# pmcbride/denoise-gan

Hardware: AMD Instinct MI355X
Metric: training images/sec, pix2pix 256x256 bs16/GPU (higher is better)
Workload: dtype fp32 (GEMMs fp16x3, operands 2^-22); 1 GPU; pix2pix train_step (train_pix2pix.py:33-71): G(x)+G(y) identity pass, D real+fake, GAN/L1/L2/TV/identity losses, D and G gradients, Keras Adam G and D; VGG19 content loss (seeded stand-in weights: ImageNet weights are a download); model=pix2pix U-Net G (54.4M) + PatchGAN D (2.77M), global_batch=16, batch_per_gpu=16, image_size=256, scale=1, parallelism=dp1, hip_graph=True, identity_pass=True

## Files before the change

denoise-gan_amd/csrc/conv.hip:

```cpp
#include "conv_plan.h"
#include "conv_tiles.h"
#include <algorithm>
#include <cstdlib>
#include <cstring>
#include <new>

namespace dg {

template <int MODE, int BM, int BN, int WGM, int WGN, bool VEC, int BK, int MINW>
__global__ void __launch_bounds__(256, MINW)
k_conv_gemm(const GemmArgs p) {
    constexpr bool A_KC = (MODE != MODE_WGRAD);
    constexpr bool B_KC = (MODE == MODE_DGRAD);
    constexpr int LDA = A_KC ? BM + 1 : BM + 4;
    constexpr int LDB = B_KC ? BN + 1 : BN + 4;
    constexpr int ASZ = BK * LDA;
    constexpr int BSZ = BK * LDB;
    constexpr int WTM = BM / WGM, WTN = BN / WGN;
    constexpr int TM = WTM / 32, TN = WTN / 32;
    static_assert(WGM * WGN == 4, "4 waves");
    static_assert(TM >= 1 && TN >= 1, "wave tile >= 32x32");
    static_assert(BK % 4 == 0 && BM >= 256 / (BK / 4) && BN >= 256 / (BK / 4), "KC loader geometry");
    static_assert(1024 / BM <= BK && 1024 / BN <= BK, "RC loader geometry");

// ... 242 lines not shown
                    *reinterpret_cast<f32x4 *>(&As[(ar_kr + AR_RPP * ip) * LDA + 4 * ar_c4]) = v;
                }
            } else {
#pragma unroll
                for (int e = 0; e < AR_NES; ++e) As[(as_kr + (256 / BM) * e) * LDA + as_c] = ra[e];
            }
        }
        if constexpr (B_KC) {
            if constexpr (VEC) {
#pragma unroll
                for (int ip = 0; ip < B_NPV; ++ip)
#pragma unroll
                    for (int q = 0; q < 4; ++q) Bs[(4 * kc_c4 + q) * LDB + kc_rr + KC_RPP * ip] = rb[4 * ip + q];
            } else {
#pragma unroll
                for (int e = 0; e < B_NES; ++e) Bs[ks_kk * LDB + ks_r0 + KS_RPP * e] = rb[e];
            }
        } else {
#pragma unroll
            for (int ip = 0; ip < BR_NP; ++ip) {
                f32x4 v = {rb[4 * ip], rb[4 * ip + 1], rb[4 * ip + 2], rb[4 * ip + 3]};
                *reinterpret_cast<f32x4 *>(&Bs[(br_kr + BR_RPP * ip) * LDB + 4 * br_c4]) = v;
            }
        }
    };

    f32x16 acc[TM][TN];
#pragma unroll
    for (int a = 0; a < TM; ++a)
#pragma unroll
        for (int b = 0; b < TN; ++b)
#pragma unroll
            for (int r = 0; r < 16; ++r) acc[a][b][r] = 0.f;

    load_tiles(kbeg);
    store_tiles(0);
    if (nk > 1) load_tiles(kbeg + BK);
    __syncthreads();

    for (int kt = 0; kt < nk; ++kt) {
        const int buf = kt & 1;
        const float *As = smem + buf * (ASZ + BSZ) + h2 * LDA + wm * WTM + l32;
        const float *Bs = smem + buf * (ASZ + BSZ) + ASZ + h2 * LDB + wn * WTN + l32;
        float af[BK / 2][TM], bf[BK / 2][TN];
#pragma unroll
        for (int s2 = 0; s2 < BK / 2; ++s2) {
#pragma unroll
            for (int a = 0; a < TM; ++a) af[s2][a] = As[2 * s2 * LDA + a * 32];
#pragma unroll
            for (int b = 0; b < TN; ++b) bf[s2][b] = Bs[2 * s2 * LDB + b * 32];
        }
        __builtin_amdgcn_sched_barrier(0);
#pragma unroll
        for (int s2 = 0; s2 < BK / 4; ++s2)
#pragma unroll
            for (int a = 0; a < TM; ++a)
#pragma unroll
                for (int b = 0; b < TN; ++b)
                    acc[a][b] = __builtin_amdgcn_mfma_f32_32x32x2f32(af[s2][a], bf[s2][b], acc[a][b], 0, 0, 0);
        __builtin_amdgcn_sched_barrier(0);
        if (kt + 1 < nk) store_tiles(buf ^ 1);
        if (kt + 2 < nk) load_tiles(kbeg + (kt + 2) * BK);
        __builtin_amdgcn_sched_barrier(0);
#pragma unroll
        for (int s2 = BK / 4; s2 < BK / 2; ++s2)
#pragma unroll
            for (int a = 0; a < TM; ++a)
#pragma unroll
                for (int b = 0; b < TN; ++b)
                    acc[a][b] = __builtin_amdgcn_mfma_f32_32x32x2f32(af[s2][a], bf[s2][b], acc[a][b], 0, 0, 0);
        __syncthreads();
    }

    static_assert(4 * 32 * 36 <= 2 * (ASZ + BSZ), "epilogue staging fits in the operand tiles");
    auto rowmap = [&](int row) __attribute__((always_inline)) -> RowPix {
        if (row >= Mrows) return RowPix{-1, -1};
        if constexpr (MODE == MODE_DGRAD) {
            int ww = row % ph.Wp; int t = row / ph.Wp; int hh = t % ph.Hp; int n = t / ph.Hp;
            return RowPix{row, (long)(n * g.H + hh * g.sh + ph.ph) * g.W + ww * g.sw + ph.pw};
        } else {
            return RowPix{row, row};
        }
    };
    conv_epilogue32<MODE, TM, TN>(p, acc, m0 + wm * WTM, n0 + wn * WTN, rowmap, phase, split, lane, smem + wid * 32 * 36);
}

template <int MODE>
__global__ void __launch_bounds__(256)
k_splitk_reduce(const GemmArgs p, int V4) {
    const ConvGeom &g = p.g;
    const int phase = blockIdx.y;
    int Mrows = p.M;
    PhaseInfo ph{};
    if constexpr (MODE == MODE_DGRAD) {
        ph = phase_info(g, phase, g.N);
        Mrows = ph.Mp;
    }
    const long plane = (long)p.M * p.N;
    const float *base = p.slab + (long)phase * p.splits * plane;
    const float ys = p.yp ? plane_scale(p) : 0.f;
    float vmax = 0.f;
    if (V4) {
        const int tpo = V4, opb = 256 / tpo;
        const int o = threadIdx.x % opb, j = threadIdx.x / opb;
        __shared__ f32x4 red[256];
        const int N4 = p.N >> 2;
        const long total = (long)Mrows * N4;
        const long step = (long)tpo * plane;
        for (long e0 = (long)blockIdx.x * opb; e0 < total; e0 += (long)gridDim.x * opb) {
            const long e = e0 + o;
            f32x4 v = {0.f, 0.f, 0.f, 0.f};
            int row = 0, col = 0;
            if (e < total) {
                row = (int)(e / N4);
                col = (int)(e - (long)row * N4) * 4;
                const float *src = base + (long)row * p.N + col + (long)j * plane;
                int s = j;
                for (; s + 3 * tpo < p.splits; s += 4 * tpo, src += 4 * step) {
                    const f32x4 a0 = *reinterpret_cast<const f32x4 *>(src);
                    const f32x4 a1 = *reinterpret_cast<const f32x4 *>(src + step);
                    const f32x4 a2 = *reinterpret_cast<const f32x4 *>(src + 2 * step);
                    const f32x4 a3 = *reinterpret_cast<const f32x4 *>(src + 3 * step);
                    v += a0;
                    v += a1;
                    v += a2;
                    v += a3;
                }
                for (; s < p.splits; s += tpo, src += step) v += *reinterpret_cast<const f32x4 *>(src);
            }
            if (tpo > 1) {
                red[threadIdx.x] = v;
                __syncthreads();
                if (j == 0)
                    for (int k = 1; k < tpo; ++k) v += red[k * opb + o];
                __syncthreads();
            }
            if (j != 0 || e >= total) continue;
            long pix;
            if constexpr (MODE == MODE_DGRAD) {
                int ww = row % ph.Wp; int t = row / ph.Wp; int hh = t % ph.Hp; int n = t / ph.Hp;
                pix = (long)(n * g.H + hh * g.sh + ph.ph) * g.W + ww * g.sw + ph.pw;
            } else {
                pix = row;
            }
            const long off = pix * p.ldc;
            f32x4 ov, mf;
#pragma unroll
            for (int q = 0; q < 4; ++q) {
                float x = v[q];
                if (p.bias) x += p.bias[col + q];
                mf[q] = epi_mask_factor(p, pix, col + q);
                ov[q] = act_fwd(x, p.act, p.alpha) * mf[q];
            }
            if (p.C) {
                f32x4 *dst = reinterpret_cast<f32x4 *>(p.C + off + col);
                if (p.beta != 0.f) ov += p.beta * (p.mask_acc ? (*dst) * mf : (*dst));
                *dst = ov;
            }
            if (p.yp) store_planes4(p.yp, p.ypC, pix, col, ov, ys);
#pragma unroll
            for (int q = 0; q < 4; ++q) vmax = fmaxf(vmax, fabsf(ov[q]));
        }
        if (p.ymax) block_atomic_absmax(p.ymax, vmax);
        return;
    }
    const long total = (long)Mrows * p.N;
    for (long e = (long)blockIdx.x * blockDim.x + threadIdx.x; e < total; e += (long)gridDim.x * blockDim.x) {
        int row = (int)(e / p.N);
        int col = (int)(e - (long)row * p.N);
        float v = 0.f;
        for (int s = 0; s < p.splits; ++s) v += base[s * plane + (long)row * p.N + col];
        long pix;
        if constexpr (MODE == MODE_DGRAD) {
            int ww = row % ph.Wp; int t = row / ph.Wp; int hh = t % ph.Hp; int n = t / ph.Hp;
            pix = (long)(n * g.H + hh * g.sh + ph.ph) * g.W + ww * g.sw + ph.pw;
        } else {
            pix = row;
        }
        const long off = pix * p.ldc;
        if (p.bias) v += p.bias[col];
        const float mf = epi_mask_factor(p, pix, col);
        v = act_fwd(v, p.act, p.alpha) * mf;
        if (p.C) {
            if (p.beta != 0.f) v += p.beta * (p.mask_acc ? p.C[off + col] * mf : p.C[off + col]);
            p.C[off + col] = v;
        }
        if (p.yp) store_planes1(p.yp, p.ypC, pix, col, v, ys);
        vmax = fmaxf(vmax, fabsf(v));
    }
    if (p.ymax) block_atomic_absmax(p.ymax, vmax);
}

constexpr int NARROW_MAX = 8;

__global__ void __launch_bounds__(256)
k_narrow_fwd(const GemmArgs p) {
    const ConvGeom &g = p.g;
    const int lane = threadIdx.x & 63;
    const int m = blockIdx.x * 4 + (threadIdx.x >> 6);
    if (m >= p.M) return;
    int wo = m % g.Wo; int t = m / g.Wo; int ho = t % g.Ho; int n = t / g.Ho;
    float acc[NARROW_MAX] = {};
    const int Co = g.Co;
    for (int i = 0; i < g.kh; ++i) {
        int hi = ho * g.sh - g.pt + i;
        if (hi < 0 || hi >= g.H) continue;
        for (int j = 0; j < g.kw; ++j) {
            int wi = wo * g.sw - g.pl + j;
            if (wi < 0 || wi >= g.W) continue;
            const float *xp = p.A + ((long)(n * g.H + hi) * g.W + wi) * p.lda;
            const float *wp = p.B + (long)(i * g.kw + j) * g.Ci * Co;
            for (int ci = lane; ci < g.Ci; ci += 64) {
                float xv = xp[ci];
#pragma unroll
                for (int co = 0; co < NARROW_MAX; ++co)
                    if (co < Co) acc[co] += xv * wp[(long)ci * Co + co];
            }
        }
    }
#pragma unroll
    for (int co = 0; co < NARROW_MAX; ++co) {
        float v = acc[co];
#pragma unroll
        for (int off = 32; off >= 1; off >>= 1) v += __shfl_xor(v, off);
        acc[co] = v;
    }
    if (lane == 0) {
        for (int co = 0; co < Co; ++co) {
            float v = acc[co];
            if (p.bias) v += p.bias[co];
            v = epi_mask(p, m, co, act_fwd(v, p.act, p.alpha));
            long off = (long)m * p.ldc + co;
            if (p.beta != 0.f) v += p.beta * p.C[off];
            p.C[off] = v;
        }
    }
}

__global__ void __launch_bounds__(256)
k_narrow_dgrad(const GemmArgs p, int w_in_lds) {
    extern __shared__ __attribute__((aligned(16))) float wl[];
    const ConvGeom &g = p.g;
    const int phase = blockIdx.y;
    PhaseInfo ph = phase_info(g, phase, g.N);
    const long wsz = (long)g.kh * g.kw * g.Ci * g.Co;
    const float *wsrc = p.B;
    if (w_in_lds) {
        for (long e = threadIdx.x; e < wsz; e += blockDim.x) wl[e] = p.B[e];
        __syncthreads();
        wsrc = wl;
    }
    const int m = blockIdx.x * blockDim.x + threadIdx.x;
    if (m >= ph.Mp) return;
    int ww = m % ph.Wp; int t = m / ph.Wp; int hh = t % ph.Hp; int n = t / ph.Hp;
    const int h = hh * g.sh + ph.ph, w = ww * g.sw + ph.pw;
    const int Ci = g.Ci, Co = g.Co;
    float acc[NARROW_MAX] = {};
    for (int a = 0; a < g.Th; ++a) {
        int i = ph.i0h + a * g.sh;
        int th = h + g.pt - i;
        if (i >= g.kh || th < 0) continue;
        int ho = th / g.sh;
        if (ho >= g.Ho) continue;
        for (int b = 0; b < g.Tw; ++b) {
            int j = ph.i0w + b * g.sw;
            int tw = w + g.pl - j;
            if (j >= g.kw || tw < 0) continue;
            int wo = tw / g.sw;
            if (wo >= g.Wo) continue;
            const float *dyp = p.A + ((long)(n * g.Ho + ho) * g.Wo + wo) * p.lda;
            const float *wp = wsrc + (long)(i * g.kw + j) * Ci * Co;
            if ((Co & 3) == 0 && (p.lda & 3) == 0) {
                for (int co = 0; co < Co; co += 4) {
                    f32x4 d = *reinterpret_cast<const f32x4 *>(dyp + co);
#pragma unroll
                    for (int ci = 0; ci < NARROW_MAX; ++ci) {
                        if (ci < Ci) {
                            const float *wr = wp + (long)ci * Co + co;
                            acc[ci] += d[0] * wr[0] + d[1] * wr[1] + d[2] * wr[2] + d[3] * wr[3];
                        }
                    }
                }
            } else {
                for (int co = 0; co < Co; ++co) {
                    float d = dyp[co];
#pragma unroll
                    for (int ci = 0; ci < NARROW_MAX; ++ci)
                        if (ci < Ci) acc[ci] += d * wp[(long)ci * Co + co];
                }
            }
        }
    }
    const long pix = (long)(n * g.H + h) * g.W + w;
    long off = pix * p.ldc;
    for (int ci = 0; ci < Ci; ++ci) {
        float v = acc[ci];
        if (p.bias) v += p.bias[ci];
        v = epi_mask(p, pix, ci, act_fwd(v, p.act, p.alpha));
        if (p.beta != 0.f) v += p.beta * p.C[off + ci];
        p.C[off + ci] = v;
    }
}


template <int CI, int TH, int TW>
__global__ void __launch_bounds__(256)
k_direct_dgrad(const GemmArgs p, int tiles_x, int tiles_y) {
    constexpr int HH = DIR_PH + TH - 1, HW = DIR_PW + TW - 1;
    __shared__ __attribute__((aligned(16))) float hal[HH * HW * DIR_CS];
    __shared__ __attribute__((aligned(16))) float wl[TH * TW * CI * DIR_CC];
    const ConvGeom &g = p.g;
    const int nph = g.sh * g.sw;
    const PhaseInfo ph = phase_info(g, blockIdx.x % nph, g.N);
    int t = blockIdx.x / nph;
    const int tx = t % tiles_x;
    t /= tiles_x;
    const int ty = t % tiles_y;
    const int n = t / tiles_y;
    const int hh0 = ty * DIR_PH, ww0 = tx * DIR_PW;
    if (hh0 >= ph.Hp || ww0 >= ph.Wp) return;
    const int oh = (ph.ph + g.pt - ph.i0h) / g.sh, ow = (ph.pw + g.pl - ph.i0w) / g.sw;
    const int ho0 = hh0 + oh - (TH - 1), wo0 = ww0 + ow - (TW - 1);
    const int lr = threadIdx.x / DIR_PW, lc = threadIdx.x % DIR_PW;
    float acc[CI];
#pragma unroll
    for (int ci = 0; ci < CI; ++ci) acc[ci] = 0.f;
    constexpr int NE = HH * HW * (DIR_CC / 4), NL = (NE + 255) / 256;
    f32x4 hv[NL];
    auto load_halo = [&](int c0) __attribute__((always_inline)) {
#pragma unroll
        for (int k = 0; k < NL; ++k) {
            const int e = threadIdx.x + 256 * k;
            hv[k] = f32x4{0.f, 0.f, 0.f, 0.f};
            if (e < NE) {
                const int q = e % (DIR_CC / 4), px = e / (DIR_CC / 4);
                const int r = px / HW, c = px - r * HW;
                const int ho = ho0 + r, wo = wo0 + c;
                if ((unsigned)ho < (unsigned)g.Ho && (unsigned)wo < (unsigned)g.Wo)
                    hv[k] = *reinterpret_cast<const f32x4 *>(p.A + ((long)(n * g.Ho + ho) * g.Wo + wo) * p.lda + c0 +
                                                             4 * q);
            }
        }
    };
    load_halo(0);
    for (int c0 = 0; c0 < g.Co; c0 += DIR_CC) {
        __syncthreads();
#pragma unroll
        for (int k = 0; k < NL; ++k) {
            const int e = threadIdx.x + 256 * k;
            if (e < NE) {
                const int q = e % (DIR_CC / 4), px = e / (DIR_CC / 4);
                *reinterpret_cast<f32x4 *>(&hal[px * DIR_CS + 4 * q]) = hv[k];
            }
        }
        for (int e = threadIdx.x; e < TH * TW * CI * DIR_CC; e += 256) {
            const int cc = e % DIR_CC, k = e / DIR_CC;
            const int ci = k % CI, tap = k / CI;
            const int i = ph.i0h + (tap / TW) * g.sh, j = ph.i0w + (tap % TW) * g.sw;
            wl[e] = (i < g.kh && j < g.kw) ? p.B[((long)(i * g.kw + j) * g.Ci + ci) * g.Co + c0 + cc] : 0.f;
        }
        __syncthreads();
        if (c0 + DIR_CC < g.Co) load_halo(c0 + DIR_CC);
#pragma unroll
        for (int a = 0; a < TH; ++a)
#pragma unroll
            for (int b = 0; b < TW; ++b) {
                const float *hp = &hal[((lr + TH - 1 - a) * HW + (lc + TW - 1 - b)) * DIR_CS];
                const float *wp = &wl[(a * TW + b) * CI * DIR_CC];
#pragma unroll
                for (int q = 0; q < DIR_CC / 4; ++q) {
                    const f32x4 d = *reinterpret_cast<const f32x4 *>(hp + 4 * q);
#pragma unroll
                    for (int ci = 0; ci < CI; ++ci) {
                        const f32x4 w = *reinterpret_cast<const f32x4 *>(wp + ci * DIR_CC + 4 * q);
                        float v = acc[ci];
                        v = fmaf(d[0], w[0], v);
                        v = fmaf(d[1], w[1], v);
                        v = fmaf(d[2], w[2], v);
                        v = fmaf(d[3], w[3], v);
                        acc[ci] = v;
                    }
                }
            }
    }
    const int hh = hh0 + lr, ww = ww0 + lc;
    if (hh >= ph.Hp || ww >= ph.Wp) return;
    const long pix = (long)(n * g.H + hh * g.sh + ph.ph) * g.W + ww * g.sw + ph.pw;
    const long off = pix * p.ldc;
#pragma unroll
    for (int ci = 0; ci < CI; ++ci) {
        float v = acc[ci];
        if (p.bias) v += p.bias[ci];
        v = epi_mask(p, pix, ci, act_fwd(v, p.act, p.alpha));
        if (p.beta != 0.f) v += p.beta * p.C[off + ci];
        p.C[off + ci] = v;
    }
}

static void launch_direct_dgrad(const GemmArgs &a, hipStream_t s) {
    const ConvGeom &g = a.g;
    const int Hp = (g.H + g.sh - 1) / g.sh, Wp = (g.W + g.sw - 1) / g.sw;
    const int tx = (Wp + DIR_PW - 1) / DIR_PW, ty = (Hp + DIR_PH - 1) / DIR_PH;
    const dim3 grid((unsigned)(g.N * tx * ty * g.sh * g.sw));
    if (g.Ci == 3 && g.Th == 3) hipLaunchKernelGGL((k_direct_dgrad<3, 3, 3>), grid, dim3(256), 0, s, a, tx, ty);
    else if (g.Ci == 3) hipLaunchKernelGGL((k_direct_dgrad<3, 2, 2>), grid, dim3(256), 0, s, a, tx, ty);
    else hipLaunchKernelGGL((k_direct_dgrad<6, 2, 2>), grid, dim3(256), 0, s, a, tx, ty);
}

constexpr int NFWD_WMAX = 8192;
constexpr long NFWD_PX_MIN_M = 4096;
template <int CO>
__global__ void __launch_bounds__(256)
k_narrow_fwd_px(const GemmArgs p) {
    __shared__ __attribute__((aligned(16))) float wl[NFWD_WMAX];
    const ConvGeom &g = p.g;
    const int ci4 = g.Ci / 4, ntap = g.kh * g.kw;
    for (int e = threadIdx.x; e < ntap * g.Ci * CO; e += 256) {
        const int q = e & 3, co = (e >> 2) % CO, rest = (e >> 2) / CO;
        const int c4 = rest % ci4, tap = rest / ci4;
        wl[e] = p.B[((long)tap * g.Ci + c4 * 4 + q) * CO + co];
    }
    __syncthreads();
    for (int m = blockIdx.x * 256 + threadIdx.x; m < p.M; m += gridDim.x * 256) {
        const int wo = m % g.Wo, t = m / g.Wo, ho = t % g.Ho, n = t / g.Ho;
        float acc[CO];
#pragma unroll
        for (int co = 0; co < CO; ++co) acc[co] = 0.f;
        for (int i = 0; i < g.kh; ++i) {
            const int hi = ho * g.sh - g.pt + i;
            if (hi < 0 || hi >= g.H) continue;
            for (int j = 0; j < g.kw; ++j) {
                const int wi = wo * g.sw - g.pl + j;
                if (wi < 0 || wi >= g.W) continue;
                const f32x4 *xp = reinterpret_cast<const f32x4 *>(p.A + ((long)(n * g.H + hi) * g.W + wi) * p.lda);
                const f32x4 *wp = reinterpret_cast<const f32x4 *>(wl) + (long)(i * g.kw + j) * ci4 * CO;
#pragma unroll 4
                for (int c = 0; c < ci4; ++c) {
                    const f32x4 x = xp[c];
#pragma unroll
                    for (int co = 0; co < CO; ++co) {
                        const f32x4 w = wp[c * CO + co];
                        acc[co] = fmaf(x[0], w[0], fmaf(x[1], w[1], fmaf(x[2], w[2], fmaf(x[3], w[3], acc[co]))));
                    }
                }
            }
        }
#pragma unroll
        for (int co = 0; co < CO; ++co) {
            float v = acc[co];
            if (p.bias) v += p.bias[co];
            v = epi_mask(p, m, co, act_fwd(v, p.act, p.alpha));
            const long off = (long)m * p.ldc + co;
            if (p.beta != 0.f) v += p.beta * p.C[off];
            p.C[off] = v;
        }
    }
}

__global__ void __launch_bounds__(256)
k_narrow_wgrad(const GemmArgs p) {
    __shared__ float red[256 * NARROW_MAX];
    const ConvGeom &g = p.g;
    const int nchunk = (g.Ci + 255) / 256;
    const int tap = blockIdx.x / nchunk;
    const int cchunk = blockIdx.x - tap * nchunk;
    int CL = 1;
    while (CL < g.Ci - cchunk * 256 && CL < 256) CL <<= 1;
    const int PL = 256 / CL;
    const int cl = threadIdx.x % CL, pl = threadIdx.x / CL;
    const int ci = cchunk * 256 + cl;
    const bool cok = ci < g.Ci;
    const int split = blockIdx.y;
    const int i = tap / g.kw, j = tap - (tap / g.kw) * g.kw;
    const int Co = g.Co;
    const int pb = split * p.kchunk, pe = min(p.K, pb + p.kchunk);
    float acc[NARROW_MAX] = {};
    constexpr int U = 4;
    int wo = (pb + pl) % g.Wo, ho = ((pb + pl) / g.Wo) % g.Ho, n = (pb + pl) / (g.Wo * g.Ho);
    auto advance = [&]() __attribute__((always_inline)) {
        wo += PL;
        if (wo >= g.Wo) {
            const int q = wo / g.Wo;
            wo -= q * g.Wo;
            ho += q;
            if (ho >= g.Ho) {
                const int q2 = ho / g.Ho;
                ho -= q2 * g.Ho;
                n += q2;
            }
        }
    };
    for (int pix0 = pb + pl; pix0 < pe; pix0 += U * PL) {
        float xv[U], dv[U][NARROW_MAX];
#pragma unroll
        for (int u = 0; u < U; ++u) {
            const int pix = pix0 + u * PL;
            xv[u] = 0.f;
#pragma unroll
            for (int co = 0; co < NARROW_MAX; ++co) dv[u][co] = 0.f;
            const int hi = ho * g.sh - g.pt + i, wi = wo * g.sw - g.pl + j, nn = n;
            advance();
            if (pix >= pe) continue;
            if (!cok || hi < 0 || hi >= g.H || wi < 0 || wi >= g.W) continue;
            xv[u] = p.A[((long)(nn * g.H + hi) * g.W + wi) * p.lda + ci];
            const float *dyp = p.B + (long)pix * p.ldb;
#pragma unroll
            for (int co = 0; co < NARROW_MAX; ++co)
                if (co < Co) dv[u][co] = dyp[co];
        }
#pragma unroll
        for (int u = 0; u < U; ++u)
#pragma unroll
            for (int co = 0; co < NARROW_MAX; ++co) acc[co] += xv[u] * dv[u][co];
    }
#pragma unroll
    for (int co = 0; co < NARROW_MAX; ++co) red[threadIdx.x * NARROW_MAX + co] = acc[co];
    __syncthreads();
    if (pl != 0 || !cok) return;
    for (int l = 1; l < PL; ++l)
#pragma unroll
        for (int co = 0; co < NARROW_MAX; ++co) acc[co] += red[(threadIdx.x + l * CL) * NARROW_MAX + co];
    const int krow = tap * g.Ci + ci;
    for (int co = 0; co < Co; ++co)
        p.slab[((long)split * p.M + krow) * p.N + co] = acc[co];
}


__global__ void __launch_bounds__(256)
k_narrow_wgrad_tile(const GemmArgs p, int nseg, float *__restrict__ part) {
    extern __shared__ __attribute__((aligned(16))) float sm[];
    const ConvGeom &g = p.g;
    const int Ci = g.Ci, KW = g.kw, KH = g.kh, Co = g.Co;
    const int CG = (Co + 3) >> 2;
    const int XW = NWT_TP + KW - 1;
    const int XE = KH * XW * Ci;
    float *xs = sm;
    f32x4 *ds = reinterpret_cast<f32x4 *>(sm + ((XE + 3) & ~3));
    const bool xv4 = (Ci & 3) == 0 && (p.lda & 3) == 0 && (((uintptr_t)p.A) & 15) == 0;
    const bool dv4 = (Co & 3) == 0 && (p.ldb & 3) == 0 && (((uintptr_t)p.B) & 15) == 0;
    const int S = KH * KW * Ci * CG;
    const int segw = (g.Wo + NWT_TP - 1) / NWT_TP;
    f32x4 acc[NWT_QMAX];
#pragma unroll
    for (int u = 0; u < NWT_QMAX; ++u) acc[u] = f32x4{0.f, 0.f, 0.f, 0.f};
    for (int seg = blockIdx.x; seg < nseg; seg += gridDim.x) {
        const int sx = seg % segw, t = seg / segw;
        const int ho = t % g.Ho, n = t / g.Ho;
        const int wo0 = sx * NWT_TP;
        if (xv4) {
            const int ci4 = Ci >> 2;
            for (int e = threadIdx.x; e < XE / 4; e += 256) {
                const int c4 = e % ci4, r = e / ci4;
                const int col = r % XW, i = r / XW;
                const int hi = ho - g.pt + i, wi = wo0 - g.pl + col;
                f32x4 v = {0.f, 0.f, 0.f, 0.f};
                if ((unsigned)hi < (unsigned)g.H && (unsigned)wi < (unsigned)g.W)
                    v = *reinterpret_cast<const f32x4 *>(p.A + ((long)(n * g.H + hi) * g.W + wi) * p.lda + 4 * c4);
                reinterpret_cast<f32x4 *>(xs)[e] = v;
            }
        } else {
            for (int e = threadIdx.x; e < XE; e += 256) {
                const int c = e % Ci, r = e / Ci;
                const int col = r % XW, i = r / XW;
                const int hi = ho - g.pt + i, wi = wo0 - g.pl + col;
                xs[e] = ((unsigned)hi < (unsigned)g.H && (unsigned)wi < (unsigned)g.W)
                            ? p.A[((long)(n * g.H + hi) * g.W + wi) * p.lda + c] : 0.f;
            }
        }
        for (int e = threadIdx.x; e < NWT_TP * CG; e += 256) {
            const int px = e / CG, cg = e - px * CG;
            const int wo = wo0 + px;
            f32x4 d = {0.f, 0.f, 0.f, 0.f};
            if (wo < g.Wo) {
                const float *dp = p.B + ((long)(n * g.Ho + ho) * g.Wo + wo) * p.ldb + 4 * cg;
                if (dv4) {
                    d = *reinterpret_cast<const f32x4 *>(dp);
                } else {
#pragma unroll
                    for (int co = 0; co < 4; ++co)
                        if (4 * cg + co < Co) d[co] = dp[co];
                }
            }
            ds[e] = d;
        }
        __syncthreads();
        const int npx = min(NWT_TP, g.Wo - wo0);
#pragma unroll
        for (int u = 0; u < NWT_QMAX; ++u) {
            const int sl = threadIdx.x + 256 * u;
            if (sl < S) {
                const int q = sl / CG, cg = sl - q * CG;
                const int tap = q / Ci, c = q - tap * Ci;
                const int i = tap / KW, j = tap - i * KW;
                const float *xr = xs + (i * XW + j) * Ci + c;
                const f32x4 *dr = ds + cg;
                f32x4 a = acc[u];
                for (int px = 0; px < npx; ++px) {
                    const float xv = xr[px * Ci];
                    const f32x4 d = dr[px * CG];
#pragma unroll
                    for (int co = 0; co < 4; ++co) a[co] = fmaf(xv, d[co], a[co]);
                }
                acc[u] = a;
            }
        }
        __syncthreads();
    }
#pragma unroll
    for (int u = 0; u < NWT_QMAX; ++u) {
        const int sl = threadIdx.x + 256 * u;
        if (sl < S) reinterpret_cast<f32x4 *>(part)[(long)blockIdx.x * S + sl] = acc[u];
    }
}

__global__ void __launch_bounds__(256)
k_narrow_wgrad_final(const GemmArgs p, int R, const float *__restrict__ part) {
    __shared__ float red[256];
    const int CG4 = 4 * ((p.N + 3) >> 2);
    const int T = p.M * CG4;
    const int ol = threadIdx.x & 15, rl = threadIdx.x >> 4;
    const int o = blockIdx.x * 16 + ol;
    float sacc = 0.f;
    if (o < T) {
#pragma unroll 8
        for (int r = rl; r < R; r += 16) sacc += part[(long)r * T + o];
    }
    red[threadIdx.x] = sacc;
    __syncthreads();
    if (rl == 0 && o < T) {
        const int q = o / CG4, co = o - q * CG4;
        if (co < p.N) {
            float t = red[ol];
            for (int l = 1; l < 16; ++l) t += red[l * 16 + ol];
            float *dst = p.C + (long)q * p.ldc + co;
            *dst = p.beta != 0.f ? t + p.beta * *dst : t;
        }
    }
}

__global__ void __launch_bounds__(256)
k_colsum_partial(const float *dy, int ld, long M, int C, long rows_per_block, float *partial) {
    __shared__ float red[256];
    int CC = 1;
    while (CC < C && CC < 64) CC <<= 1;
    const int RL = 256 / CC;
    const int cl = threadIdx.x % CC, rl = threadIdx.x / CC;
    const int c = blockIdx.y * CC + cl;
    long r0 = (long)blockIdx.x * rows_per_block;
    long r1 = min(M, r0 + rows_per_block);
    float s = 0.f;
    if (c < C) {
#pragma unroll 4
        for (long r = r0 + rl; r < r1; r += RL) s += dy[r * ld + c];
    }
    red[threadIdx.x] = s;
    __syncthreads();
    if (rl != 0 || c >= C) return;
    for (int l = 1; l < RL; ++l) s += red[l * CC + cl];
    partial[(long)c * gridDim.x + blockIdx.x] = s;
}
__global__ void __launch_bounds__(256) k_colsum_final(const float *partial, int nblk, int C, float *out, float beta) {
    __shared__ float red[256];
    const int c = blockIdx.x;
    float s = 0.f;
    for (int b = threadIdx.x; b < nblk; b += 256) s += partial[(long)c * nblk + b];
    red[threadIdx.x] = s;
    __syncthreads();
    for (int o = 128; o > 0; o >>= 1) {
        if ((int)threadIdx.x < o) red[threadIdx.x] += red[threadIdx.x + o];
        __syncthreads();
    }
    if (threadIdx.x == 0) out[c] = red[0] + (beta != 0.f ? beta * out[c] : 0.f);
}

__global__ void __launch_bounds__(256)
k_transpose(const float *__restrict__ src, int R, int Cc, float *__restrict__ dst, int Rp) {
    const long total = (long)Rp * Cc;
    for (long e = (long)blockIdx.x * blockDim.x + threadIdx.x; e < total; e += (long)gridDim.x * blockDim.x) {
        int c = (int)(e / Rp);
        int r = (int)(e - (long)c * Rp);
        dst[e] = r < R ? src[(long)r * Cc + c] : 0.f;
    }
}
// ... 828 lines not shown
```

denoise-gan_amd/csrc/conv_small.hip:

```cpp
#include "conv_impl.h"
#include <algorithm>

namespace dg {

constexpr int SC_BN = 64;
constexpr int SC_CH = 8;

__host__ __device__ constexpr int sc_up(int x, int r) { return x + (((r - x) % 32) + 32) % 32; }

template <int CI, int P, int KW = 4, int S = 2>
struct Strip {
    static_assert((KW == 4 && S == 2) || (KW == 3 && S == 1), "4x4 stride 2 or 3x3 stride 1");
    static constexpr int COLS = S == 2 ? P + 1 : P + KW - 1;
    static constexpr int PAR = S == 2 ? sc_up(COLS * CI, 2 * CI) : 0;
    static constexpr int ROW = S == 2 ? sc_up(2 * PAR, 4 * CI) : sc_up(COLS * CI, 4 * CI);
    static constexpr int SIZE = 4 * ROW;
    static constexpr int WL = S * P + KW - S;
    static constexpr int NLOAD = 4 * WL * CI;
    static constexpr int KHALF = 2 * KW * CI;
    __host__ __device__ static constexpr int tap(int k) {
        return S == 2 ? ((k / CI) >> 2) * ROW + (((k / CI) & 3) & 1) * PAR + (((k / CI) & 3) >> 1) * CI + k % CI
                      : ((k / CI) / KW) * ROW + ((k / CI) % KW) * CI + k % CI;
    }
    __host__ __device__ static constexpr int pos(int row, int wl, int ci) {
        return S == 2 ? row * ROW + (wl & 1) * PAR + (wl >> 1) * CI + ci : row * ROW + wl * CI + ci;
    }
};

template <int CI, int P, int NTHR, int KW = 4, int ST = 2>
__device__ __forceinline__ void strip_fetch(const GemmArgs &p, int n, int ho, int wo0, int tid,
                                            float (&r)[(Strip<CI, P, KW, ST>::NLOAD + NTHR - 1) / NTHR]) {
    using S = Strip<CI, P, KW, ST>;
    const ConvGeom &g = p.g;
    const int h0 = ST * ho - g.pt, w0 = ST * wo0 - g.pl;
#pragma unroll
    for (int q = 0; q < (S::NLOAD + NTHR - 1) / NTHR; ++q) {
        const int e = tid + q * NTHR;
        const int row = e / (S::WL * CI), rem = e - row * (S::WL * CI);
        const int wl = rem / CI, ci = rem - wl * CI;
        const int h = h0 + row, w = w0 + wl;
        const bool ok = ((S::NLOAD % NTHR) == 0 || e < S::NLOAD) && (unsigned)h < (unsigned)g.H &&
                        (unsigned)w < (unsigned)g.W;
        r[q] = ok ? p.A[((long)(n * g.H + h) * g.W + w) * p.lda + ci] : 0.f;
    }
}

template <int CI, int P, int NTHR, int KW = 4, int ST = 2>
__device__ __forceinline__ void strip_store(float *s, int tid,
                                            const float (&r)[(Strip<CI, P, KW, ST>::NLOAD + NTHR - 1) / NTHR]) {
    using S = Strip<CI, P, KW, ST>;
#pragma unroll
    for (int q = 0; q < (S::NLOAD + NTHR - 1) / NTHR; ++q) {
        const int e = tid + q * NTHR;
        if ((S::NLOAD % NTHR) != 0 && q == (S::NLOAD + NTHR - 1) / NTHR - 1 && e >= S::NLOAD) break;
        const int row = e / (S::WL * CI), rem = e - row * (S::WL * CI);
        const int wl = rem / CI, ci = rem - wl * CI;
        s[S::pos(row, wl, ci)] = r[q];
    }
}

constexpr int SC_STAGE = 32 * 36;
struct SmallEpi {
    f32x4 bias;
    f32x4 z[4], c[4];
};
__device__ __forceinline__ bool sc_vec(const void *ptr, int ld) { return ((ld & 3) == 0) && ((((uintptr_t)ptr) & 15) == 0); }
__device__ __forceinline__ f32x4 sc_ld4(const float *a, bool vec) {
    return vec ? *reinterpret_cast<const f32x4 *>(a) : f32x4{a[0], a[1], a[2], a[3]};
}
__device__ __forceinline__ void small_epi_load(const GemmArgs &p, int rbase, int cbase, int lane, SmallEpi &e) {
    const int col = cbase + (lane & 7) * 4;
#pragma unroll
    for (int i = 0; i < 4; ++i) {
        const long pix = rbase + (lane >> 3) + 8 * i;
        const bool in = pix < p.M;
        if (p.mz) e.z[i] = in ? sc_ld4(p.mz + pix * p.ldmz + col, sc_vec(p.mz, p.ldmz)) : f32x4{0.f, 0.f, 0.f, 0.f};
        if (p.beta != 0.f) e.c[i] = in ? sc_ld4(p.C + pix * p.ldc + col, sc_vec(p.C, p.ldc)) : f32x4{0.f, 0.f, 0.f, 0.f};
    }
}
template <bool XL>
__device__ __forceinline__ void small_fwd_epilogue(const GemmArgs &p, const f32x16 &acc, int rbase, int cbase,
                                                   float *stage, int lane, const SmallEpi &e, float &vmax, float ys) {
    const int l32 = lane & 31, h2 = lane >> 5;
#pragma unroll
    for (int r = 0; r < 16; ++r) stage[((r & 3) + 8 * (r >> 2) + 4 * h2) * 36 + l32] = acc[r];
    const bool cvec = sc_vec(p.C, p.ldc);
    const int col = cbase + (lane & 7) * 4;
#pragma unroll
    for (int i = 0; i < 4; ++i) {
        const int row = (lane >> 3) + 8 * i;
        f32x4 o = *reinterpret_cast<const f32x4 *>(stage + row * 36 + (lane & 7) * 4);
        const long pix = rbase + row;
        if (pix >= p.M) continue;
        if (p.bias) o += e.bias;
#pragma unroll
        for (int q = 0; q < 4; ++q) o[q] = act_fwd(o[q], p.act, p.alpha);
        if constexpr (XL) {
            if (p.mz) {
#pragma unroll
                for (int q = 0; q < 4; ++q) o[q] *= act_grad_from_out(e.z[i][q], p.mact, p.malpha);
            }
            if (p.beta != 0.f) o += p.beta * e.c[i];
        }
        float *dst = p.C + pix * p.ldc + col;
        if (!p.C) {
        } else if (cvec) {
            *reinterpret_cast<f32x4 *>(dst) = o;
        } else {
#pragma unroll
            for (int q = 0; q < 4; ++q) dst[q] = o[q];
        }
        if (p.yp) store_planes4(p.yp, p.ypC, pix, col, o, ys);
        if (p.ymax) {
#pragma unroll
            for (int q = 0; q < 4; ++q) vmax = fmaxf(vmax, fabsf(o[q]));
        }
    }
}

template <int CI, int P, bool XL, int KW = 4, int ST = 2>
__global__ void __launch_bounds__(128 * (P / 32))
k_small_fwd(const GemmArgs p) {
    using S = Strip<CI, P, KW, ST>;
    constexpr int KH = S::KHALF;
    constexpr int KTOT = KW * KW * CI;
    constexpr int CH = KH % SC_CH == 0 ? SC_CH : 6;
    static_assert(KH % CH == 0, "operand chunks");
    constexpr int NTHR = 128 * (P / 32);
    constexpr int NL = (S::NLOAD + NTHR - 1) / NTHR;
    __shared__ __attribute__((aligned(16))) float strip[2][S::SIZE];
    __shared__ __attribute__((aligned(16))) float stage[2 * (P / 32)][SC_STAGE];
    const ConvGeom &g = p.g;
    const int tid = threadIdx.x, lane = tid & 63, wid = tid >> 6;
    const int sub = wid >> 1, nt = wid & 1;
    const int l32 = lane & 31, h2 = lane >> 5;
    const int col0 = blockIdx.y * SC_BN + nt * 32;
    float wr[KH];
#pragma unroll
    for (int s = 0; s < KH; ++s) wr[s] = s + h2 * KH < KTOT ? p.B[(long)(s + h2 * KH) * p.ldb + col0 + l32] : 0.f;
    const int segs = g.Wo / P;
    const int ntiles = g.N * g.Ho * segs;
    const int abase = h2 * 2 * S::ROW + (sub * 32 + l32) * CI;
    SmallEpi epi;
    if (p.bias) epi.bias = sc_ld4(p.bias + col0 + (lane & 7) * 4, false);
    float pre[NL];
    float vmax = 0.f;
    const X3Raw ysr = x3_raw(p.ys_m, p.ys_g, p.ys_c);
    int t = blockIdx.x;
    if (t >= ntiles) return;
    {
        const int row = t / segs, n = row / g.Ho;
        strip_fetch<CI, P, NTHR, KW, ST>(p, n, row - n * g.Ho, (t - row * segs) * P, tid, pre);
        strip_store<CI, P, NTHR, KW, ST>(strip[0], tid, pre);
    }
    __syncthreads();
    for (int it = 0; t < ntiles; t += gridDim.x, ++it) {
        const int tn = t + gridDim.x;
        const int row = t / segs;
        const int rbase = row * g.Wo + (t - row * segs) * P + sub * 32;
        if constexpr (XL) small_epi_load(p, rbase, col0, lane, epi);
        {
            const int tf = tn < ntiles ? tn : t;
            const int rown = tf / segs, n = rown / g.Ho;
            strip_fetch<CI, P, NTHR, KW, ST>(p, n, rown - n * g.Ho, (tf - rown * segs) * P, tid, pre);
        }
        const float *sb = strip[it & 1] + abase;
        f32x16 acc;
#pragma unroll
        for (int r = 0; r < 16; ++r) acc[r] = 0.f;
        float a[2][CH];
#pragma unroll
        for (int u = 0; u < CH; ++u) a[0][u] = sb[S::tap(u)];
#pragma unroll
        for (int c = 0; c < KH / CH; ++c) {
            if (c + 1 < KH / CH) {
#pragma unroll
                for (int u = 0; u < CH; ++u) a[(c + 1) & 1][u] = sb[S::tap((c + 1) * CH + u)];
            }
#pragma unroll
            for (int u = 0; u < CH; ++u)
                acc = __builtin_amdgcn_mfma_f32_32x32x2f32(a[c & 1][u], wr[c * CH + u], acc, 0, 0, 0);
        }
        strip_store<CI, P, NTHR, KW, ST>(strip[(it + 1) & 1], tid, pre);
        small_fwd_epilogue<XL>(p, acc, rbase, col0, stage[wid], lane, epi, vmax, x3_raw_scale(ysr, F16X3_XS));
        __syncthreads();
    }
    if (p.ymax) block_atomic_absmax(p.ymax, vmax);
}

template <int CI, int P>
__global__ void __launch_bounds__(128 * ((16 * CI + 31) / 32))
k_small_wgrad(const GemmArgs p, int rows_per_block) {
    using S = Strip<CI, P>;
    constexpr int M = 16 * CI;
    constexpr int MT = (M + 31) / 32;
    constexpr int NTHR = 128 * MT;
    constexpr int NL = (S::NLOAD + NTHR - 1) / NTHR;
    constexpr int LDB = SC_BN + 4;
    constexpr int NB = (P * SC_BN / 4 + NTHR - 1) / NTHR;
    __shared__ __attribute__((aligned(16))) float strip[2][S::SIZE];
    __shared__ __attribute__((aligned(16))) float Bs[2][P * LDB];
    const ConvGeom &g = p.g;
    const int tid = threadIdx.x, lane = tid & 63, wid = tid >> 6;
    const int mt = wid >> 1, nt = wid & 1;
    const int l32 = lane & 31, h2 = lane >> 5;
    const int split = blockIdx.x;
    const int n0 = blockIdx.y * SC_BN;
    const int segs = g.Wo / P;
    const int k0 = split * rows_per_block * segs;
    const int k1 = min(g.N * g.Ho, (split + 1) * rows_per_block) * segs;
    const int m = mt * 32 + l32;
    const int mm = m < M ? m : 0;
    const int tp = mm / CI, ci = mm - tp * CI;
    const int abase = (tp >> 2) * S::ROW + (tp & 1) * S::PAR + ((tp & 3) >> 1) * CI + ci + h2 * CI;
    const int bbase = h2 * LDB + nt * 32 + l32;
    const bool bvec = ((p.ldb & 3) == 0) && ((((uintptr_t)p.B) & 15) == 0);
    float pre[NL];
    f32x4 preb[NB];
    auto fetch = [&](int kt) {
        const int row = kt / segs, wo0 = (kt - row * segs) * P, n = row / g.Ho;
        strip_fetch<CI, P, NTHR>(p, n, row - n * g.Ho, wo0, tid, pre);
        const long pix0 = (long)row * g.Wo + wo0;
#pragma unroll
        for (int q = 0; q < NB; ++q) {
            const int e = tid + q * NTHR;
            const int k = e / (SC_BN / 4), c = (e - k * (SC_BN / 4)) * 4;
            f32x4 v = {0.f, 0.f, 0.f, 0.f};
            if (e < P * SC_BN / 4) {
                const float *src = p.B + (pix0 + k) * p.ldb + n0 + c;
                if (bvec) v = *reinterpret_cast<const f32x4 *>(src);
                else v = f32x4{src[0], src[1], src[2], src[3]};
            }
            preb[q] = v;
        }
    };
    auto store = [&](int buf) {
        strip_store<CI, P, NTHR>(strip[buf], tid, pre);
#pragma unroll
        for (int q = 0; q < NB; ++q) {
            const int e = tid + q * NTHR;
            if (e >= P * SC_BN / 4) break;
            const int k = e / (SC_BN / 4), c = (e - k * (SC_BN / 4)) * 4;
            *reinterpret_cast<f32x4 *>(&Bs[buf][k * LDB + c]) = preb[q];
        }
    };
    f32x16 acc;
#pragma unroll
    for (int r = 0; r < 16; ++r) acc[r] = 0.f;
    if (k0 < k1) {
        fetch(k0);
        store(0);
    }
    __syncthreads();
    for (int kt = k0, it = 0; kt < k1; ++kt, ++it) {
        if (kt + 1 < k1) fetch(kt + 1);
        const float *sa = strip[it & 1] + abase;
        const float *sb = Bs[it & 1] + bbase;
        float a[2][SC_CH], b[2][SC_CH];
#pragma unroll
        for (int u = 0; u < SC_CH; ++u) {
            a[0][u] = sa[2 * u * CI];
            b[0][u] = sb[2 * u * LDB];
        }
#pragma unroll
        for (int c = 0; c < P / 2 / SC_CH; ++c) {
            if (c + 1 < P / 2 / SC_CH) {
#pragma unroll
                for (int u = 0; u < SC_CH; ++u) {
                    const int st = (c + 1) * SC_CH + u;
                    a[(c + 1) & 1][u] = sa[2 * st * CI];
                    b[(c + 1) & 1][u] = sb[2 * st * LDB];
                }
            }
#pragma unroll
            for (int u = 0; u < SC_CH; ++u)
                acc = __builtin_amdgcn_mfma_f32_32x32x2f32(a[c & 1][u], b[c & 1][u], acc, 0, 0, 0);
        }
        if (kt + 1 < k1) store((it + 1) & 1);
        __syncthreads();
    }
    const int col = n0 + nt * 32 + l32;
#pragma unroll
    for (int r = 0; r < 16; ++r) {
        const int row = mt * 32 + (r & 3) + 8 * (r >> 2) + 4 * h2;
        if (row >= M) continue;
        if (p.splits > 1) {
            p.slab[((long)split * p.M + row) * p.N + col] = acc[r];
        } else {
            float *dst = p.C + (long)row * p.ldc + col;
            *dst = p.beta != 0.f ? acc[r] + p.beta * *dst : acc[r];
        }
    }
}

bool small_conv_ok(const ConvGeom &g, int mode, int lda) {
    (void)lda;
    if (mode != MODE_FWD && mode != MODE_WGRAD) return false;
    if (g.kh == 3 && g.kw == 3 && g.sh == 1 && g.sw == 1)
        return mode == MODE_FWD && g.Ci == 3 && g.Co % SC_BN == 0 && g.Wo % 32 == 0;
    return g.kh == 4 && g.kw == 4 && g.sh == 2 && g.sw == 2 && (g.Ci == 3 || g.Ci == 6) && g.Co % SC_BN == 0 &&
           g.Wo % 32 == 0;
}

int small_wgrad_rows_per_block(const ConvGeom &g) {
    const int rows = g.N * g.Ho, cols = g.Co / SC_BN;
    const int want = std::max(1, 512 / cols);
    return std::max(1, (rows + want - 1) / want);
}

template <int CI, int P, int KW = 4, int ST = 2>
static void launch_small(int mode, const GemmArgs &a, int rows_per_block, hipStream_t s) {
    const ConvGeom &g = a.g;
    if (mode == MODE_WGRAD) {
        if constexpr (KW == 4) {
            const int rows = g.N * g.Ho;
            const dim3 grid((unsigned)((rows + rows_per_block - 1) / rows_per_block), (unsigned)(g.Co / SC_BN));
            hipLaunchKernelGGL((k_small_wgrad<CI, P>), grid, dim3(128 * ((16 * CI + 31) / 32)), 0, s, a, rows_per_block);
        }
    } else {
        static int resident = 0;
        if (!resident) {
            int per_cu = 0, dev = 0, cus = 256;
            if (hipOccupancyMaxActiveBlocksPerMultiprocessor(&per_cu, k_small_fwd<CI, P, true, KW, ST>, 128 * (P / 32),
                                                             0) != hipSuccess ||
                per_cu < 1)
                per_cu = 1;
            if (hipGetDevice(&dev) != hipSuccess ||
                hipDeviceGetAttribute(&cus, hipDeviceAttributeMultiprocessorCount, dev) != hipSuccess)
                cus = 256;
            resident = per_cu * cus;
        }
        const int ntiles = g.N * g.Ho * (g.Wo / P);
        const int cols = g.Co / SC_BN;
        const dim3 grid((unsigned)std::max(1, std::min(ntiles, resident / cols)), (unsigned)cols);
        if (a.mz || a.beta != 0.f) hipLaunchKernelGGL((k_small_fwd<CI, P, true, KW, ST>), grid, dim3(128 * (P / 32)), 0, s, a);
        else hipLaunchKernelGGL((k_small_fwd<CI, P, false, KW, ST>), grid, dim3(128 * (P / 32)), 0, s, a);
    }
}

void launch_small_conv(int mode, const GemmArgs &a, int rows_per_block, hipStream_t s) {
    const bool p64 = a.g.Wo % 64 == 0;
    if (a.g.kh == 3) {
        if (p64) launch_small<3, 64, 3, 1>(mode, a, rows_per_block, s);
        else launch_small<3, 32, 3, 1>(mode, a, rows_per_block, s);
    } else if (a.g.Ci == 3) {
        if (p64) launch_small<3, 64>(mode, a, rows_per_block, s);
        else launch_small<3, 32>(mode, a, rows_per_block, s);
    } else {
        if (p64) launch_small<6, 64>(mode, a, rows_per_block, s);
        else launch_small<6, 32>(mode, a, rows_per_block, s);
    }
}

}
```

Measured before the change: 1050 images/s.

## Read direct-dgrad weights via scalar constant loads and size small-conv grids per variant

The direct dgrad kernel no longer stages weights into LDS. It reads them through the constant address space as wave-uniform scalar loads and feeds them into inline-asm v_fmac chains that take SGPR operands. Taps that fall outside the kernel use a zero-stride pointer to a zero constant array. This removes an LDS fill, a large shared buffer and the LDS weight reads, at the cost of many SGPRs and a CI%3 restriction. Separately, the small-conv forward launcher now caches its occupancy-based grid size for each template variant (with or without mask/beta), instead of always using the masked variant's occupancy.

```diff
diff --git a/denoise-gan_amd/csrc/conv.hip b/denoise-gan_amd/csrc/conv.hip
--- a/denoise-gan_amd/csrc/conv.hip
+++ b/denoise-gan_amd/csrc/conv.hip
@@ -568,13 +568,28 @@
     }
 }
 
+#define dir_as4 __attribute__((address_space(4)))
+typedef const float dir_as4 dir_wf;
+__constant__ const float DIR_ZERO_W[DIR_CC] = {};
+__device__ __forceinline__ void dir_fma3x4(float &a0, float &a1, float &a2, const f32x4 &d, const f32x4 &w0,
+                                           const f32x4 &w1, const f32x4 &w2) {
+    asm("v_fmac_f32_e32 %0, %7, %3\n\tv_fmac_f32_e32 %1, %11, %3\n\tv_fmac_f32_e32 %2, %15, %3\n\t"
+        "v_fmac_f32_e32 %0, %8, %4\n\tv_fmac_f32_e32 %1, %12, %4\n\tv_fmac_f32_e32 %2, %16, %4\n\t"
+        "v_fmac_f32_e32 %0, %9, %5\n\tv_fmac_f32_e32 %1, %13, %5\n\tv_fmac_f32_e32 %2, %17, %5\n\t"
+        "v_fmac_f32_e32 %0, %10, %6\n\tv_fmac_f32_e32 %1, %14, %6\n\tv_fmac_f32_e32 %2, %18, %6"
+        : "+v"(a0), "+v"(a1), "+v"(a2)
+        : "v"(d[0]), "v"(d[1]), "v"(d[2]), "v"(d[3]), "s"(w0[0]), "s"(w0[1]), "s"(w0[2]), "s"(w0[3]), "s"(w1[0]),
+          "s"(w1[1]), "s"(w1[2]), "s"(w1[3]), "s"(w2[0]), "s"(w2[1]), "s"(w2[2]), "s"(w2[3]));
+}
 
 template <int CI, int TH, int TW>
 __global__ void __launch_bounds__(256)
 k_direct_dgrad(const GemmArgs p, int tiles_x, int tiles_y) {
     constexpr int HH = DIR_PH + TH - 1, HW = DIR_PW + TW - 1;
+    static_assert(CI % 3 == 0, "chains run in groups of three (dir_fma3x4)");
+    constexpr int QS = CI <= 3 ? 4 : 2;
+    typedef float wvec __attribute__((ext_vector_type(4 * QS), aligned(4)));
     __shared__ __attribute__((aligned(16))) float hal[HH * HW * DIR_CS];
-    __shared__ __attribute__((aligned(16))) float wl[TH * TW * CI * DIR_CC];
     const ConvGeom &g = p.g;
     const int nph = g.sh * g.sw;
     const PhaseInfo ph = phase_info(g, blockIdx.x % nph, g.N);
@@ -619,12 +634,6 @@
                 *reinterpret_cast<f32x4 *>(&hal[px * DIR_CS + 4 * q]) = hv[k];
             }
         }
-        for (int e = threadIdx.x; e < TH * TW * CI * DIR_CC; e += 256) {
-            const int cc = e % DIR_CC, k = e / DIR_CC;
-            const int ci = k % CI, tap = k / CI;
-            const int i = ph.i0h + (tap / TW) * g.sh, j = ph.i0w + (tap % TW) * g.sw;
-            wl[e] = (i < g.kh && j < g.kw) ? p.B[((long)(i * g.kw + j) * g.Ci + ci) * g.Co + c0 + cc] : 0.f;
-        }
         __syncthreads();
         if (c0 + DIR_CC < g.Co) load_halo(c0 + DIR_CC);
 #pragma unroll
@@ -632,19 +641,27 @@
 #pragma unroll
             for (int b = 0; b < TW; ++b) {
                 const float *hp = &hal[((lr + TH - 1 - a) * HW + (lc + TW - 1 - b)) * DIR_CS];
-                const float *wp = &wl[(a * TW + b) * CI * DIR_CC];
-#pragma unroll
-                for (int q = 0; q < DIR_CC / 4; ++q) {
-                    const f32x4 d = *reinterpret_cast<const f32x4 *>(hp + 4 * q);
-#pragma unroll
-                    for (int ci = 0; ci < CI; ++ci) {
-                        const f32x4 w = *reinterpret_cast<const f32x4 *>(wp + ci * DIR_CC + 4 * q);
-                        float v = acc[ci];
-                        v = fmaf(d[0], w[0], v);
-                        v = fmaf(d[1], w[1], v);
-                        v = fmaf(d[2], w[2], v);
-                        v = fmaf(d[3], w[3], v);
-                        acc[ci] = v;
+                const int i = ph.i0h + a * g.sh, j = ph.i0w + b * g.sw;
+                const bool in = i < g.kh && j < g.kw;
+                dir_wf *wp = in ? (dir_wf *)(p.B + (long)(i * g.kw + j) * CI * g.Co + c0) : (dir_wf *)DIR_ZERO_W;
+                const int wstr = in ? g.Co : 0;
+#pragma unroll
+                for (int q0 = 0; q0 < DIR_CC / 4; q0 += QS) {
+                    wvec wv[CI];
+#pragma unroll
+                    for (int ci = 0; ci < CI; ++ci) wv[ci] = *reinterpret_cast<const wvec dir_as4 *>(wp + ci * wstr + 4 * q0);
+#pragma unroll
+                    for (int qq = 0; qq < QS; ++qq) {
+                        const f32x4 d = *reinterpret_cast<const f32x4 *>(hp + 4 * (q0 + qq));
+#pragma unroll
+                        for (int c = 0; c < CI; c += 3) {
+                            f32x4 w[3];
+#pragma unroll
+                            for (int u = 0; u < 3; ++u)
+                                w[u] = f32x4{wv[c + u][4 * qq], wv[c + u][4 * qq + 1], wv[c + u][4 * qq + 2],
+                                             wv[c + u][4 * qq + 3]};
+                            dir_fma3x4(acc[c], acc[c + 1], acc[c + 2], d, w[0], w[1], w[2]);
+                        }
                     }
                 }
             }
diff --git a/denoise-gan_amd/csrc/conv_small.hip b/denoise-gan_amd/csrc/conv_small.hip
--- a/denoise-gan_amd/csrc/conv_small.hip
+++ b/denoise-gan_amd/csrc/conv_small.hip
@@ -318,22 +318,25 @@
             hipLaunchKernelGGL((k_small_wgrad<CI, P>), grid, dim3(128 * ((16 * CI + 31) / 32)), 0, s, a, rows_per_block);
         }
     } else {
-        static int resident = 0;
-        if (!resident) {
+        static int resident[2] = {0, 0};
+        const int xl = (a.mz || a.beta != 0.f) ? 1 : 0;
+        if (!resident[xl]) {
             int per_cu = 0, dev = 0, cus = 256;
-            if (hipOccupancyMaxActiveBlocksPerMultiprocessor(&per_cu, k_small_fwd<CI, P, true, KW, ST>, 128 * (P / 32),
-                                                             0) != hipSuccess ||
-                per_cu < 1)
-                per_cu = 1;
+            const hipError_t e =
+                xl ? hipOccupancyMaxActiveBlocksPerMultiprocessor(&per_cu, k_small_fwd<CI, P, true, KW, ST>,
+                                                                  128 * (P / 32), 0)
+                   : hipOccupancyMaxActiveBlocksPerMultiprocessor(&per_cu, k_small_fwd<CI, P, false, KW, ST>,
+                                                                  128 * (P / 32), 0);
+            if (e != hipSuccess || per_cu < 1) per_cu = 1;
             if (hipGetDevice(&dev) != hipSuccess ||
                 hipDeviceGetAttribute(&cus, hipDeviceAttributeMultiprocessorCount, dev) != hipSuccess)
                 cus = 256;
-            resident = per_cu * cus;
+            resident[xl] = per_cu * cus;
         }
         const int ntiles = g.N * g.Ho * (g.Wo / P);
         const int cols = g.Co / SC_BN;
-        const dim3 grid((unsigned)std::max(1, std::min(ntiles, resident / cols)), (unsigned)cols);
-        if (a.mz || a.beta != 0.f) hipLaunchKernelGGL((k_small_fwd<CI, P, true, KW, ST>), grid, dim3(128 * (P / 32)), 0, s, a);
+        const dim3 grid((unsigned)std::max(1, std::min(ntiles, resident[xl] / cols)), (unsigned)cols);
+        if (xl) hipLaunchKernelGGL((k_small_fwd<CI, P, true, KW, ST>), grid, dim3(128 * (P / 32)), 0, s, a);
         else hipLaunchKernelGGL((k_small_fwd<CI, P, false, KW, ST>), grid, dim3(128 * (P / 32)), 0, s, a);
     }
 }
```

Result: no change. 1052 images/s, median of 6 (+0.2%).
